# UBCMOCCA/mocca_envs

Hardware: AMD Instinct MI355X
Metric: env-steps/sec, Walker3DCustomEnv-v0 @ 4096 envs, 1/2/4/8 MI355X (higher is better)
Workload: dtype f32; 1 GPU; Walker3DCustomEnv-v0, 4096 envs/GPU, flat ground, U(-1,1) action tape, auto-reset; max_rows=48, max_contacts=12, envs_per_gpu=4096, parallelism=independent env shards x1, no collective, preroll_steps=5904

## Files before the change

mocca_envs_amd/csrc/mocca_api.hip:

```cpp
#include <hip/hip_runtime.h>

#include <cmath>
#include <cstdio>
#include <cstring>
#include <memory>
#include <new>
#include <string>
#include <utility>
#include <vector>

#include "mocca.h"
#include "mocca_kernels.h"
#include "mocca_optim.h"
#include "mocca_policy.h"
#include "mocca_ppo.h"
#include "mocca_render.h"
#include "mocca_rollout.h"
#include "mocca_scan.h"

using namespace mocca;

extern "C" size_t mocca_r32_args_sizeof(void);
extern "C" int mocca_r32_max_rows(void);
extern "C" int mocca_r32_max_contacts(void);
// ... 23 lines not shown
    const uint32_t r = task[(size_t)e * MOCCA_TASK_WORDS + MOCCA_TW_LAST_ROWS];
    atomicAdd(&hist[63 - (r > 63u ? 63u : r)], 1);
  }
  __syncthreads();
  if (t == 0) {
    int acc = 0;
    for (int k = 0; k < 64; ++k) { start[k] = acc; acc += hist[k]; }
  }
  __syncthreads();
  for (int e = t; e < n; e += 1024) {
    const uint32_t r = task[(size_t)e * MOCCA_TASK_WORDS + MOCCA_TW_LAST_ROWS];
    order[atomicAdd(&start[63 - (r > 63u ? 63u : r)], 1)] = e;
  }
}

template <class T>
class DevBuf {
  T* p_ = nullptr;

 public:
  DevBuf() = default;
  DevBuf(DevBuf&& o) noexcept : p_(std::exchange(o.p_, nullptr)) {}
  DevBuf& operator=(DevBuf&& o) noexcept { swap(o); return *this; }
  ~DevBuf() { reset(); }
  void reset() {
    if (p_) (void)hipFree(p_);
    p_ = nullptr;
  }
  void swap(DevBuf& o) noexcept { std::swap(p_, o.p_); }
  hipError_t alloc(size_t count, bool zero) {
    reset();
    hipError_t e = hipMalloc(&p_, count * sizeof(T));
    if (e != hipSuccess) { p_ = nullptr; return e; }
    if (zero && (e = hipMemset(p_, 0, count * sizeof(T))) != hipSuccess) reset();
    return e;
  }
  T* get() const { return p_; }
  operator T*() const { return p_; }
};

struct mocca_ctx {
  MoccaModel model;
  int task_id = 0, n_envs = 0, device = 0, obs_dim = 0;
  DevBuf<MoccaModel> d_model;
  int topo = 0;
  DevBuf<float> d_dyn;
  DevBuf<uint32_t> d_task;
  DevBuf<float> d_terrain;
  int auto_reset = 0, eval_mode = 0, random_pose = 1, curriculum = 0, host_retarget = 0, env_offset = 0, random_reward = 0;
  float gain = 1.0f;
  bool compact = false;
  bool wide = false;
  int force_full = 0;
  int persist_warm = 0;
  int pace = -18;
  DevBuf<unsigned long long> d_pace_acc;
  DevBuf<float> d_ep_ret;
  float *ep_masks = nullptr, *ep_bad = nullptr, *ep_totals = nullptr;
  char* ep_rec = nullptr;
  int ep_slots = 0;
  size_t ep_stride = 0;
  uint32_t ep_serial = 1;
  int order_every = 0;
  int order_age = 0;
  DevBuf<int32_t> d_order;
  bool gain_pending = false;
  float* final_obs = nullptr;
  DevBuf<float> d_pvec[3];
  bool pvec_on[3] = {false, false, false};
  const float* tape = nullptr;
  int tape_n = 0;
  int32_t* dbg = nullptr;
  int prio = MOCCA_PRIO_T1 + 64 * MOCCA_PRIO_T2 + 4096 * MOCCA_PRIO_T3;
  uint64_t seed = 0;
  DevBuf<float> d_traj;
  int traj_n = 0;
  double traj_tmax = 0.0, traj_cstep = 0.0;
  DevBuf<float> d_hf;
  int hf_rows = 0, hf_cols = 0;
  float hf_scale = 0.0f;
  float hf_zmin = 0.0f, hf_zmax = 0.0f;
  DevBuf<float> d_scenes;
  int scenes_cap = 0;
  DevBuf<float> d_scan_pts;
  int scan_n = 0;
  float scan_above = 0.0f, scan_drop = 0.0f;
  DevBuf<float> d_ctrl_image;
  DevBuf<int32_t> d_ctrl_layers;
  mocca_ctrl::ControllerArgs ctrl{};
  DevBuf<float> d_robot_state;
  DevBuf<float> d_base_act;
  DevBuf<float> d_base_val;
  DevBuf<float> d_ctrl_norm;
  DevBuf<float> d_pol_image;
  DevBuf<int32_t> d_pol_layers;
  mocca_pol::PolicyArgs pol{};
  mocca_pol::RepackArgs pol_repack{};
  size_t pol_n_base = 0;
  bool pol_filled = false;
  int pol_tail_row = 0;
  std::vector<int32_t> pol_table;
  int pol_wt_off[mocca_ppo::PPO_MAX_TABLE] = {};
  DevBuf<int32_t> d_pol_sym_perm;
  DevBuf<float> d_pol_sym_sign;
  DevBuf<int32_t> d_pol_ml_perm;
  DevBuf<float> d_pol_ml_sign;
// ... 286 lines not shown
  if ((e = h->d_dyn.alloc(n * DYN_STRIDE, false)) != hipSuccess) return fail("hipMalloc(state)", e);
  if ((e = h->d_task.alloc(n * MOCCA_TASK_WORDS, false)) != hipSuccess) return fail("hipMalloc(task)", e);
  if ((e = h->d_terrain.alloc(n * TERRAIN_STRIDE, true)) != hipSuccess) return fail("hipMalloc(terrain)", e);
  if ((e = h->d_pace_acc.alloc(1, true)) != hipSuccess) return fail("hipMalloc(pace samples)", e);
  {
    std::vector<uint32_t> tmp(n * MOCCA_TASK_WORDS);
    const float one = 1.0f;
    uint32_t one_bits; std::memcpy(&one_bits, &one, 4);
    for (size_t i = 0; i < n; ++i) {
      tmp[i * MOCCA_TASK_WORDS + MOCCA_TW_EPISODE] = (uint32_t)-1;
      tmp[i * MOCCA_TASK_WORDS + MOCCA_TW_APPLIED_GAIN] = one_bits;
    }
    if ((e = hipMemcpy(h->d_task, tmp.data(), tmp.size() * sizeof(uint32_t), hipMemcpyHostToDevice)) != hipSuccess) return fail("hipMemcpy(task)", e);
  }
  {
    std::vector<float> tmp(n * DYN_STRIDE);
    for (size_t i = 0; i < n; ++i) tmp[i * DYN_STRIDE + 6] = 1.0f;
    if ((e = hipMemcpy(h->d_dyn, tmp.data(), tmp.size() * sizeof(float), hipMemcpyHostToDevice)) != hipSuccess) return fail("hipMemcpy(state)", e);
  }
  *out = h.release();
  return MOCCA_OK;
} catch (const std::bad_alloc&) { return out_of_host_memory(nullptr, "mocca_create"); }

int mocca_destroy(mocca_handle h) {
  delete h;
  return MOCCA_OK;
}

int mocca_n_envs(mocca_handle h) { return h ? h->n_envs : MOCCA_E_ARG; }
int mocca_obs_dim(mocca_handle h) { return h ? h->obs_dim : MOCCA_E_ARG; }
int mocca_act_dim(mocca_handle h) {
  if (!h) return MOCCA_E_ARG;
  return h->task_id == MOCCA_TASK_CASSIE ? h->model.n_ctrl - 2 : h->model.n_joints;
}
int mocca_plan_dim(mocca_handle h) {
  if (!h) return MOCCA_E_ARG;
  if (h->task_id != MOCCA_TASK_WALKER3D_PLANNER) { h->err = "mocca_plan_dim: only the planner task takes plans"; return MOCCA_E_ARG; }
  return mocca_ctrl::CTRL_PLAN;
}
int mocca_state_dim(mocca_handle h) { return h ? MOCCA_STATE_DIM(h->model.n_joints, h->model.n_slots) : MOCCA_E_ARG; }

static StepArgs make_args(mocca_handle h) {
  StepArgs a{};
  a.model = h->d_model; a.dyn = h->d_dyn; a.task = h->d_task; a.terrain = h->d_terrain;
  a.n_envs = h->n_envs; a.obs_dim = h->obs_dim;
  a.auto_reset = h->auto_reset; a.eval_mode = h->eval_mode; a.random_pose = h->random_pose; a.curriculum = h->curriculum;
  a.host_retarget = h->host_retarget; a.env_offset = h->env_offset; a.random_reward = h->random_reward;
  a.seed_lo = (uint32_t)h->seed; a.seed_hi = (uint32_t)(h->seed >> 32);
  a.curriculum_v = h->pvec_on[0] ? h->d_pvec[0].get() : nullptr;
  a.eval_mode_v = h->pvec_on[1] ? h->d_pvec[1].get() : nullptr;
  a.gain_v = h->pvec_on[2] ? h->d_pvec[2].get() : nullptr;
  a.gain = h->gain;
  a.dbg = h->dbg;
  a.prio = h->prio;
  a.traj = h->d_traj; a.traj_n = h->traj_n; a.traj_tmax = h->traj_tmax; a.traj_cstep = h->traj_cstep;
  a.final_obs = h->final_obs;
  a.persist_warm = h->persist_warm;
  a.pace = h->pace;
  a.pace_acc = h->d_pace_acc;
  a.ep_ret = h->d_ep_ret; a.ep_masks = h->ep_masks; a.ep_bad = h->ep_bad; a.ep_totals = h->ep_totals;
  a.hf = h->d_hf; a.hf_rows = h->hf_rows; a.hf_cols = h->hf_cols; a.hf_scale = h->hf_scale;
  a.robot_state = h->d_ctrl_image ? h->d_robot_state.get() : nullptr;
  return a;
}
static int flush_pending(mocca_handle h, hipStream_t s) {
  if (!h->gain_pending) return MOCCA_OK;
  launch_per_env(set_task_word_kernel, h, s, h->d_task, MOCCA_TW_APPLIED_GAIN, nullptr, h->gain, 1, h->n_envs);
  HIP_TRY(h, hipGetLastError());
  h->gain_pending = false;
  return MOCCA_OK;
}
static int need_heightfield(mocca_handle h, const char* who, const char* when) {
  if (h->task_id != MOCCA_TASK_WALKER3D_PLANNER || h->d_hf) return MOCCA_OK;
  h->err = std::string(who) + "the planner task needs mocca_set_heightfield " + when;
  return MOCCA_E_ARG;
}
static mocca_rdr::HeightField heightfield_record(mocca_handle h) {
  if (h->task_id != MOCCA_TASK_WALKER3D_PLANNER) return mocca_rdr::HeightField{nullptr, 0, 0, 0.0f, 0.0f, 0.0f};
  return mocca_rdr::HeightField{h->d_hf, h->hf_rows, h->hf_cols, h->hf_scale, h->hf_zmin, h->hf_zmax};
}
static int need_attachments(mocca_handle h) {
  if (h->task_id == MOCCA_TASK_CASSIE && h->model.cassie_mode != MOCCA_CASSIE_PLAIN && !h->d_traj) {
    h->err = "this Cassie blob (cassie_mode != 0) needs mocca_set_trajectory before reset / step / observe";
    return MOCCA_E_ARG;
  }
  return need_heightfield(h, "", "before reset / step / observe");
}

int mocca_reset(mocca_handle h, const uint8_t* mask_dev, uint64_t seed, float* obs_dev, void* stream) {
  if (!h || !obs_dev) return MOCCA_E_ARG;
  if (need_attachments(h) != MOCCA_OK) return MOCCA_E_ARG;
  h->seed = seed;
  DeviceGuard guard(h->device);
  StepArgs a = make_args(h);
  a.mask = mask_dev; a.obs = obs_dev;
  hipStream_t s = (hipStream_t)stream;
  if (int rc = flush_pending(h, s)) return rc;
  if (h->tape) {
    a.tape = h->tape; a.tape_n = h->tape_n;
    launch_taped_reset(h->topo, h->task_id, h->n_envs, s, a);
  } else {
    dispatch<LaunchReset>(h->topo, h->task_id, h->n_envs, s, a);
  }
  HIP_TRY(h, hipGetLastError());
  return MOCCA_OK;
}

// ... 306 lines not shown
}
int mocca_set_task(mocca_handle h, const uint32_t* task_dev, void* stream) {
  if (!h || !task_dev) return MOCCA_E_ARG;
  DeviceGuard guard(h->device);
  h->gain_pending = false;
  HIP_TRY(h, hipMemcpyAsync(h->d_task, task_dev, (size_t)h->n_envs * MOCCA_TASK_WORDS * 4, hipMemcpyDeviceToDevice, (hipStream_t)stream));
  return MOCCA_OK;
}
int mocca_get_terrain(mocca_handle h, float* terrain_dev, void* stream) {
  if (!h || !terrain_dev) return MOCCA_E_ARG;
  DeviceGuard guard(h->device);
  HIP_TRY(h, hipMemcpyAsync(terrain_dev, h->d_terrain, (size_t)h->n_envs * TERRAIN_STRIDE * 4, hipMemcpyDeviceToDevice, (hipStream_t)stream));
  return MOCCA_OK;
}
int mocca_set_terrain(mocca_handle h, const float* terrain_dev, void* stream) {
  if (!h || !terrain_dev) return MOCCA_E_ARG;
  DeviceGuard guard(h->device);
  HIP_TRY(h, hipMemcpyAsync(h->d_terrain, terrain_dev, (size_t)h->n_envs * TERRAIN_STRIDE * 4, hipMemcpyDeviceToDevice, (hipStream_t)stream));
  return MOCCA_OK;
}

int mocca_set_param(mocca_handle h, int param_id, double value) {
  if (!h) return MOCCA_E_ARG;
  switch (param_id) {
    case MOCCA_PARAM_AUTO_RESET: h->auto_reset = value != 0; break;
    case MOCCA_PARAM_EVAL_MODE: h->eval_mode = value != 0; h->pvec_on[1] = false; break;
    case MOCCA_PARAM_CURRICULUM: h->curriculum = (int)value < 0 ? 0 : ((int)value > 9 ? 9 : (int)value); h->pvec_on[0] = false; break;
    case MOCCA_PARAM_APPLIED_GAIN:
      h->gain = (float)value; h->pvec_on[2] = false; h->gain_pending = true;
      break;
    case MOCCA_PARAM_RANDOM_POSE: h->random_pose = value != 0; break;
    case MOCCA_PARAM_HOST_RETARGET: h->host_retarget = value != 0; break;
    case MOCCA_PARAM_SEED: h->seed = (uint64_t)value; break;
    case MOCCA_PARAM_ENV_OFFSET: h->env_offset = (int)value; break;
    case MOCCA_PARAM_ISSUE_PRIORITY:
      if (value < 0 || value >= 262144) { h->err = "MOCCA_PARAM_ISSUE_PRIORITY is t1 + 64 t2 + 4096 t3 with each threshold in 0..63"; return MOCCA_E_ARG; }
      h->prio = (int)value;
      break;
    case MOCCA_PARAM_RANDOM_REWARD:
      if (value != 0 && value != 1 && value != 2) { h->err = "MOCCA_PARAM_RANDOM_REWARD is 0, 1 or 2"; return MOCCA_E_ARG; }
      h->random_reward = (int)value; break;
    case MOCCA_PARAM_PERSIST_IMPULSES: h->persist_warm = value != 0; break;
    case MOCCA_PARAM_PACE_TICKS:
      if (value < -64 || value > 1e9) { h->err = "MOCCA_PARAM_PACE_TICKS is a tick count > 0, 0 (off) or -k (self-calibrating, k / 16 of the mean wave time, k <= 64)"; return MOCCA_E_ARG; }
      h->pace = (int)value; break;
    case MOCCA_PARAM_ORDER_EVERY:
      if (value < 0 || value > 1e6) { h->err = "MOCCA_PARAM_ORDER_EVERY is a step count >= 0"; return MOCCA_E_ARG; }
      h->order_every = (int)value; h->order_age = h->order_every;
      if (h->order_every > 0 && !h->d_order) {
        DeviceGuard guard(h->device);
        HIP_TRY(h, h->d_order.alloc((size_t)h->n_envs, false));
      }
      break;
    case MOCCA_PARAM_KERNEL_VARIANT:
      if (value != 0 && value != 1 && value != 2) { h->err = "MOCCA_PARAM_KERNEL_VARIANT is 0 (automatic), 1 (force the 48-row instance) or 2 (force the 64-row instance)"; return MOCCA_E_ARG; }
      if (value == 1 && h->wide) { h->err = "MOCCA_PARAM_KERNEL_VARIANT = 1: this blob needs the 64-row instance (caps beyond 48 rows / 12 contacts, or sweep_alternate)"; return MOCCA_E_ARG; }
      h->force_full = (int)value; break;
    default: h->err = "unknown parameter id"; return MOCCA_E_ARG;
  }
  return MOCCA_OK;
}

int mocca_set_param_v(mocca_handle h, int param_id, const float* values_dev, int broadcast, void* stream) {
  if (!h || !values_dev) return MOCCA_E_ARG;
  const int slot = param_id == MOCCA_PARAM_CURRICULUM ? 0 : param_id == MOCCA_PARAM_EVAL_MODE ? 1 : param_id == MOCCA_PARAM_APPLIED_GAIN ? 2 : -1;
  if (slot < 0) { h->err = "this parameter has no per-env form"; return MOCCA_E_ARG; }
  DeviceGuard guard(h->device);
  if (!h->d_pvec[slot]) HIP_TRY(h, h->d_pvec[slot].alloc((size_t)h->n_envs, false));
  hipStream_t s = (hipStream_t)stream;
  launch_per_env(copy_param_kernel, h, s, h->d_pvec[slot], values_dev, broadcast != 0, h->n_envs);
  HIP_TRY(h, hipGetLastError());
  if (slot == 2) {
    h->gain_pending = false;
    launch_per_env(set_task_word_kernel, h, s, h->d_task, MOCCA_TW_APPLIED_GAIN, h->d_pvec[slot], 0.0f, 0, h->n_envs);
    HIP_TRY(h, hipGetLastError());
  }
  h->pvec_on[slot] = true;
  return MOCCA_OK;
}

static mocca_rdr::SceneArgs scene_args(mocca_handle h) {
  mocca_rdr::SceneArgs a{};
  a.model = h->d_model; a.dyn = h->d_dyn; a.task = h->d_task; a.terrain = h->d_terrain;
  a.dyn_stride = DYN_STRIDE; a.terrain_stride = TERRAIN_STRIDE; a.task_id = h->task_id;
  return a;
}

int mocca_get_link_frames(mocca_handle h, float* frames_dev, void* stream) {
  if (!h || !frames_dev) return MOCCA_E_ARG;
  DeviceGuard guard(h->device);
  mocca_rdr::launch_link_frames((hipStream_t)stream, scene_args(h), h->n_envs, frames_dev);
  HIP_TRY(h, hipGetLastError());
  return MOCCA_OK;
}

int mocca_render(mocca_handle h, const int32_t* env_ids_dev, int n_views, const float* cameras_dev, int width, int height, uint8_t* rgb_dev,
                 float* depth_dev, int32_t* id_dev, void* stream) try {
  if (!h) return MOCCA_E_ARG;
  if (!env_ids_dev || !cameras_dev) { h->err = "mocca_render: env_ids_dev and cameras_dev must not be NULL"; return MOCCA_E_ARG; }
  if (n_views < 1 || n_views > 65535) { h->err = "mocca_render: n_views must be 1 .. 65535"; return MOCCA_E_ARG; }
  if (width < 1 || height < 1 || width > MOCCA_RENDER_MAX_SIZE || height > MOCCA_RENDER_MAX_SIZE) {
    h->err = "mocca_render: width and height must be 1 .. " + std::to_string(MOCCA_RENDER_MAX_SIZE); return MOCCA_E_ARG;
  }
  if (need_heightfield(h, "mocca_render: ", "first") != MOCCA_OK) return MOCCA_E_ARG;
  DeviceGuard guard(h->device);
  hipStream_t s = (hipStream_t)stream;
  std::vector<int32_t> ids((size_t)n_views);
  HIP_TRY(h, hipMemcpyAsync(ids.data(), env_ids_dev, ids.size() * sizeof(int32_t), hipMemcpyDeviceToHost, s));
  HIP_TRY(h, hipStreamSynchronize(s));
  for (int v = 0; v < n_views; ++v)
// ... 611 lines not shown
```

mocca_envs_amd/csrc/mocca_device.h:

```cpp
#pragma once

#include <hip/hip_runtime.h>
#include <stdint.h>

#include "mocca_model.h"
#include "mocca_philox.h"
#include "topo_walker3d.h"
#include "topo_cassie.h"
#include "topo_walker2d.h"
#include "topo_crab2d.h"
#include "topo_laikago.h"

#define DI __device__ __forceinline__

#ifndef MOCCA_NS
#define MOCCA_NS mocca
#endif
#ifndef MOCCA_MAXR
#define MOCCA_MAXR 48
#endif
#ifndef MOCCA_COMPACT
#define MOCCA_COMPACT 0
#endif

// ... 1177 lines not shown
    nc += __popcll(hm);
    n_self += __popcll(hm);
    if (nc > maxc) nc = maxc;
  }
  STAMP(14);
  if (dbg && lane == 0) {
    dbg[3] = (int32_t)(unsigned)am; dbg[4] = (int32_t)(unsigned)(am >> 32); dbg[7] = n_self;
  }
  *nc_out = nc;
  *nc_wanted = n_terrain + n_self;
  return fl;
}

template <class T, int TT>
DI void delassus_dots(const float* L, const float* X, int oc, int onr, int tmax, float* v) {
  if constexpr (TT <= MAXR / 2) {
    if (TT > tmax) return;
    const unsigned o = (unsigned)(oc + 28 * TT);
    const unsigned ow = o - (unsigned)onr;
    const float* Jr = L + L_J + (int)(o < ow ? o : ow);
    float s;
    if constexpr (T::NCLOS > 0) {
      float s0 = 0, s1 = 0;
#pragma unroll
      for (int d = 0; d + 1 < T::ND; d += 2) { s0 += Jr[d] * X[d]; s1 += Jr[d + 1] * X[d + 1]; }
      if constexpr (T::ND & 1) s0 += Jr[T::ND - 1] * X[T::ND - 1];
      s = s0 + s1;
    } else {
      s = 0;
#pragma unroll
      for (int d = 0; d < T::ND; ++d) s += Jr[d] * X[d];
    }
    v[TT] = s;
    pin1(v[TT]);
    delassus_dots<T, TT + 1>(L, X, oc, onr, tmax, v);
  }
}
template <int TT>
DI void delassus_store(float* L, int c, int nr, int tmax, const float* v) {
  if constexpr (TT <= MAXR / 2) {
    if (TT > tmax) return;
    const unsigned r0 = (unsigned)(c + TT), rw = r0 - (unsigned)nr;
    const int rho = (int)(r0 < rw ? r0 : rw);
    if (TT == 0) {
      L[L_A + (MAXR + 1) * c] = 0.0f;
    } else {
      L[L_A + __mul24(MAXR, rho) + c] = v[TT];
      L[L_A + __mul24(MAXR, c) + rho] = v[TT];
    }
    delassus_store<TT + 1>(L, c, nr, tmax, v);
  }
}

template <int RR>
DI void pgs_visit(float as, float& y, float& lam, float lo0) {
  const float nl_ = __builtin_amdgcn_fmed3f(y, lo0, 1e30f);
  const float dl = readlane(nl_ - lam, RR);
  lam = commit_lane<RR>(nl_, lam);
  y = fmaf(-as, dl, y);
}
template <int RR>
DI void pgs_visit_friction(float as, float& y, float& lam, float lm) {
  const float nl_ = __builtin_amdgcn_fmed3f(y, -lm, lm);
  const float dl = readlane(nl_ - lam, RR);
  lam = commit_lane<RR>(nl_, lam);
  y = fmaf(-as, dl, y);
}
template <int A>
DI float commit_pair(float v, float old) {
  float r;
  unsigned long long m;
  asm("s_mov_b64 %1, 0\n\ts_bitset1_b64 %1, %4\n\ts_bitset1_b64 %1, %5\n\tv_cndmask_b32 %0, %2, %3, %1"
      : "=v"(r), "=&s"(m) : "v"(old), "v"(v), "n"(A), "n"(A + 1));
  return r;
}
template <int A, int B>
DI void pgs_visit_cone(float asA, float asB, float& y, float& lam, float lm) {
  static_assert(B == A + 1 && A % 2 == 0, "the pair must share a DPP quad");
  const float y2 = y * y;
  const float r2 = y2 + dpp_mov<0xB1>(y2);
  const float sc = fminf(1.0f, lm * rsq(r2));
  const float nl_ = y * sc;
  const float dl = nl_ - lam;
  const float dA = readlane(dl, A), dB = readlane(dl, B);
  lam = commit_pair<A>(nl_, lam);
  y = fmaf(-asA, dA, y);
  y = fmaf(-asB, dB, y);
}
constexpr int fric_lane(int i, int s) { return MAXR - 2 - 2 * i + s; }
#ifdef MOCCA_PGS_REG_ROWS
template <class T> struct PgsWin { static constexpr int ROWS = MOCCA_PGS_REG_ROWS, CONTACTS = MOCCA_PGS_REG_CONTACTS; };
#else
template <class T> struct PgsWin { static constexpr int ROWS = T::NCLOS > 0 ? 24 : 12, CONTACTS = T::NCLOS > 0 ? 8 : 4; };
#endif
template <int PGS_REG_ROWS, int PGS_REG_CONTACTS, int I, bool CONE>
DI void pgs_friction_rows(const float* Acol, const float* af, float a0, float a1, float b0, float b1, int nc, float& y, float& lam, float invdiag, float lm,
                          unsigned long long fpos) {
  if constexpr (I < MAXC) {
    if (I >= nc) return;
    constexpr int IN = I + 2 < MAXC ? I + 2 : MAXC - 1;
    float n0 = 0.0f, n1 = 0.0f;
    if constexpr (I + 2 >= PGS_REG_CONTACTS) {
      if (I + 2 < nc) { n0 = Acol[MAXR * fric_lane(IN, 0)]; n1 = Acol[MAXR * fric_lane(IN, 1)]; }
    }
    const float gA = I < PGS_REG_CONTACTS ? af[2 * (I < PGS_REG_CONTACTS ? I : 0)] : a0 * invdiag;
    const float gB = I < PGS_REG_CONTACTS ? af[2 * (I < PGS_REG_CONTACTS ? I : 0) + 1] : a1 * invdiag;
// ... 63 lines not shown
  else if (nr > (prio & 63)) __builtin_amdgcn_s_setprio(1);
  else __builtin_amdgcn_s_setprio(0);
}
#ifndef MOCCA_PACE_ROWUNIT
#define MOCCA_PACE_ROWUNIT 2
#endif
#ifndef MOCCA_PACE_SHIFT
#define MOCCA_PACE_SHIFT 4
#endif
constexpr int PACE_TICK_SHIFT = 6;
enum : int { L_T0 = L_BASE + 13, L_PACE = L_BASE + 14, L_KEEPWARM = L_BASE + 15  };
constexpr unsigned PACE_CNT_BITS = 24, PACE_WINDOW = 128;
DI void pace_start(const StepArgs& a, float* L, int lane, int pace) {
  if (lane == 0) {
    int p16 = pace >> PACE_TICK_SHIFT;
    if (pace < 0) {
      const unsigned long long v = __hip_atomic_load(a.pace_acc, __ATOMIC_RELAXED, __HIP_MEMORY_SCOPE_AGENT);
      const unsigned cnt = (unsigned)v & ((1u << PACE_CNT_BITS) - 1u);
      p16 = cnt > 0u ? (int)((float)(v >> PACE_CNT_BITS) / (float)cnt * (float)(-pace) * 0.0625f) : 0;
    }
    L[L_PACE] = __int_as_float(p16);
    if (pace != 0) L[L_T0] = __uint_as_float((unsigned)__builtin_amdgcn_s_memtime());
  }
}
DI void pace_finish(const StepArgs& a, const float* L, int lane, int pace) {
  if (pace < 0 && lane == 0 && (blockIdx.x % 61u) == 0u) {
    const unsigned el = ((unsigned)__builtin_amdgcn_s_memtime() - __float_as_uint(L[L_T0])) >> PACE_TICK_SHIFT;
    const unsigned long long old = atomicAdd(a.pace_acc, ((unsigned long long)el << PACE_CNT_BITS) | 1ull);
    if (((unsigned)old & ((1u << PACE_CNT_BITS) - 1u)) + 1u == PACE_WINDOW) {
      const unsigned long long sum = (old >> PACE_CNT_BITS) + el;
      atomicAdd(a.pace_acc, 0ull - (((sum >> 1) << PACE_CNT_BITS) | (unsigned long long)(PACE_WINDOW / 2)));
    }
  }
}
DI bool pace_on(const float* L) { return uni(__float_as_int(L[L_PACE])) > 0; }
DI void pace_checkpoint(const float* L, int done, int total) {
  const unsigned p16 = (unsigned)uni(__float_as_int(L[L_PACE]));
  if (p16 == 0u) return;
  const unsigned el = (unsigned)__builtin_amdgcn_s_memtime() - (unsigned)uni(__float_as_int(L[L_T0]));
  const unsigned lhs = (el >> PACE_TICK_SHIFT) * (unsigned)total, r = p16 * (unsigned)done;
  if (lhs > r + (r >> MOCCA_PACE_SHIFT)) __builtin_amdgcn_s_setprio(3);
  else if (lhs > r) __builtin_amdgcn_s_setprio(2);
  else if (lhs > r - (r >> MOCCA_PACE_SHIFT)) __builtin_amdgcn_s_setprio(1);
  else __builtin_amdgcn_s_setprio(0);
}
DI void dbg_fold_step(int32_t* dbg, int lane) {
  if (dbg && lane == 0) {
    unsigned long long h = ((unsigned long long)(unsigned)dbg[17] << 32) | (unsigned)dbg[16];
#pragma unroll 1
    for (int w = 0; w < 12; ++w) h = (h ^ (unsigned long long)(unsigned)dbg[w]) * 0x9E3779B97F4A7C15ull;
    dbg[16] = (int32_t)(unsigned)h; dbg[17] = (int32_t)(unsigned)(h >> 32); dbg[18] += 1;
  }
}
template <class T>
DI void solve_constraints(ModelP M, float* L, int lane, int nc_found, int nc_wanted, unsigned long long ppk, int32_t* dbg, const float* Afac, int prio, int& rows_out) {
  const bool keep_warm = uni(__float_as_int(L[L_KEEPWARM])) != 0;
  STAMP_BEGIN;
  const float dt = unif(M->dt), idt = rcp(dt);
  const int maxr = uni(M->max_rows);
  int nl;
  {
    bool act = false;
    if (lane < 2 * T::NJ) {
      const int b = 1 + (lane >> 1), side = lane & 1;
      const float q = L[L_Q + b];
      const float gap = side == 0 ? q - M->jlo[b] : M->jhi[b] - q;
      const float vel = (side == 0 ? 1.0f : -1.0f) * L[L_NU + 5 + b];
      act = M->limit_at_violation ? !(gap > 0.0f) : gap + dt * vel < M->limit_slack;
    }
    const unsigned long long lm = __ballot(act);
    const int rk = lane_rank(lm);
    if (act && rk < maxr) reinterpret_cast<int*>(L)[L_ROWD + rk] = lane;
    nl = uni(__popcll(lm));
    if (dbg && lane == 0) {
      dbg[5] = (int32_t)(unsigned)lm; dbg[6] = (int32_t)(unsigned)(lm >> 32);
      const int nfix = 3 * T::NCLOS + ((T::NCLOS > 0 && M->planar) ? 3 : 0), mc = M->max_contacts;
      const int wanted = nl + nfix + 3 * nc_wanted;
      dbg[12] += nc_wanted > mc ? 1 : 0;
      dbg[13] += nl + nfix + 3 * (nc_wanted < mc ? nc_wanted : mc) > maxr ? 1 : 0;
      dbg[14] += 1;
      if (wanted > dbg[15]) dbg[15] = wanted;
    }
    if (nl > maxr) nl = maxr;
  }
  constexpr int NCL = 3 * T::NCLOS;
  const int NFIX = NCL + ((T::NCLOS > 0 && uni(M->planar)) ? 3 : 0);
  int nc = uni(nc_found);
  if (nc > (maxr - nl - NFIX) / 3) nc = (maxr - nl - NFIX) / 3;
  if (nc < 0) nc = 0;
  const int nr = nl + NFIX + 3 * nc;
  if (dbg && lane == 0) { dbg[0] = nr; dbg[1] = nl; dbg[2] = nc; }
  if (!pace_on(L)) set_issue_priority(nr, prio);
  rows_out = nr;
  wsync();
  STAMP(16);
  if (nr == 0) {
    if (dbg && lane == 0) { dbg[8] = 0; dbg[9] = 0; dbg[10] = 0; dbg[11] = 0; }
    if (keep_warm && lane < T::NSLOT) L[L_WARM + lane] = 0.0f;
    wsync();
    return;
  }
  const int r = lane;
  const int r_fr = nl + NFIX + nc;
  const int row_gap = MAXR - nr;
  const bool is_fric = r >= MAXR - 2 * nc && r < MAXR;
  const bool has_row = r < r_fr || is_fric;
  const int ci = is_fric ? (MAXR - 1 - r) >> 1 : r - nl - NFIX;
  int kind = -1, ba = 0, bb = -1, jl = -1, slot = -1;
  float F[6] = {0, 0, 0, 0, 0, 0}, sgn = 0, bias = 0, cfm = 0, lam = 0, mu = 0;
// ... 129 lines not shown
      for (int i = 0; i < 6; ++i) pb[i] += U[i] * uu;
      if (valid) Jrow[5 + jj] += jb;
      w += jb * L[L_NU + 5 + jj];
      pub[k] = uu * L[L_SV + SVS * jj + SV_INVD];
      pin6(pb); pin1(pub[k]); pin1(w);
    }
  } else {
#pragma unroll
    for (int k = 0; k < T::MAXD; ++k) pub[k] = 0.0f;
  }
  STAMP(19);
  int l2off = 0;
  asm volatile("" : "+v"(l2off));
  l2off &= ~3;
  const float* L2 = L + l2off;
  float a0[6];
  {
    float rhs[6];
#pragma unroll
    for (int i = 0; i < 6; ++i) {
      const float jb = F[i] * sa - F2[i] * sb;
      Jrow[i] = jb;
      w += jb * L[L_NU + i];
      rhs[i] = jb - (pa[i] + pb[i]);
    }
    chol6_solve(Afac, rhs, a0);
#pragma unroll
    for (int i = 0; i < 6; ++i) X[i] = a0[i];
  }
  {
    float acc[T::NB][6];
#pragma unroll
    for (int i = 0; i < 6; ++i) acc[0][i] = a0[i];
#pragma unroll
    for (int b = 1; b < T::NB; ++b) {
      const int p = T::parent(b);
      float S[6], U[6];
#pragma unroll
      for (int i = 0; i < 6; ++i) { S[i] = L2[L_SV + SVS * b + i]; U[i] = L2[L_SV + SVS * b + SV_V + i]; }
      const int dpos = T::depth(b) - 1;
      float ub = __uint_as_float(__float_as_uint(pu[dpos]) & (unsigned)__builtin_amdgcn_sbfe((int)ma, b, 1));
      if (two_paths) ub += __uint_as_float(__float_as_uint(pub[dpos]) & (unsigned)__builtin_amdgcn_sbfe((int)mb, b, 1));
      const float qdd = ub - dot6(U, acc[p]);
      X[5 + b] = qdd;
#pragma unroll
      for (int i = 0; i < 6; ++i) acc[b][i] = acc[p][i] + S[i] * qdd;
      pin6(acc[b]); pin1(X[5 + b]);
    }
  }
  STAMP(6);
  wsync();
  const int lc = has_row ? dense : MAXR - 1;
  float diag;
  {
    float av[MAXR / 2 + 1];
    const int cc = has_row ? dense : 0, tmax = nr >> 1;
    delassus_dots<T, 0>(L, X, 28 * cc, 28 * nr, tmax, av);
    diag = has_row ? av[0] : 1.0f;
    wsync();
    if (has_row) delassus_store<0>(L, cc, nr, tmax, av);
  }
  const float invdiag = diag + cfm > 1e-12f ? rcp(diag + cfm) : 0.0f;
  wsync();
  STAMP(7);
  if (__ballot(lam != 0.0f) != 0ull) {
    int rr = nl + NFIX;
    const int rend = nl + NFIX + nc;
#pragma unroll 1
    for (; rr + 2 <= rend; rr += 2) {
      const float g0 = L[L_A + MAXR * rr + lc], g1 = L[L_A + MAXR * rr + MAXR + lc];
      w += g0 * readlane(lam, rr); w += g1 * readlane(lam, rr + 1);
    }
    if (rr < rend) w += L[L_A + MAXR * rr + lc] * readlane(lam, rr);
  }
  STAMP(20);
  const int iters = uni(M->n_iters);
  const bool cone = uni(M->friction_cone) != 0;
  const float lo0 = kind == 3 ? -1e30f : 0.0f;
  const float* Acol = L + L_A + lc;
  const float* Acol_fr = Acol - MAXR * row_gap;
  const int nrow_lane = is_fric ? nl + NFIX + ci : 0;
  float y = (bias - w) * invdiag;
  constexpr int PGS_REG_ROWS = PgsWin<T>::ROWS, PGS_REG_CONTACTS = PgsWin<T>::CONTACTS;
  static_assert(PGS_REG_ROWS % 4 == 0 && PGS_REG_ROWS <= MAXR && PGS_REG_CONTACTS <= MAXC, "register window of the solver");
  float ar[PGS_REG_ROWS], af[2 * PGS_REG_CONTACTS];
#pragma unroll
  for (int k = 0; k < PGS_REG_ROWS; ++k) ar[k] = Acol[MAXR * k] * invdiag;
#pragma unroll
  for (int k = 0; k < PGS_REG_CONTACTS; ++k) {
    af[2 * k] = 0.0f; af[2 * k + 1] = 0.0f;
    if (k < nc) { af[2 * k] = Acol_fr[MAXR * fric_lane(k, 0)] * invdiag; af[2 * k + 1] = Acol_fr[MAXR * fric_lane(k, 1)] * invdiag; }
  }
  unsigned long long clamp_sig = 0ull, clamp_last = 0ull;
  const int nnc = nl + NFIX;
  const bool alt = ALT_SWEEPS && uni(M->sweep_alternate) != 0 && nnc > 1;
#pragma unroll 1
  for (int it = 0; it < iters; ++it) {
    int rf = r_fr, ncc = nc;
    asm volatile("" : "+s"(rf), "+s"(ncc));
    bool fwd = true;
    if constexpr (ALT_SWEEPS) {
      if (alt && !(it & 1)) {
        int nn = nnc;
        asm volatile("" : "+s"(nn));
        pgs_reverse_rows(Acol, nn, lane, y, lam, invdiag, lo0);
        pgs_fixed_rows_from<PGS_REG_ROWS, 0>(Acol, ar, nn, rf, y, lam, invdiag, lo0);
        fwd = false;
// ... 131 lines not shown
  }
  wsync();
}

template <class T, int TASK>
DI ContactFlags substep(ModelP M, float* L, int lane, const float* ter, int next_step_index,
                        unsigned long long ppk, int32_t* dbg, int prio, int& rows_out,
                        const HeightFieldArgs hfa = HeightFieldArgs{nullptr, 0, 0, 0.0f}, int sidx = 0, int nsub = 1, int* cover_out = nullptr) {
  const int per0 = 64 + MOCCA_PACE_ROWUNIT * rows_out, done0 = sidx * per0, total = nsub * per0;
  STAMP(30);
  stage_joints<T>(M, L, lane);
  STAMP(29);
  int nc = 0, nc_wanted = 0;
  float Afac[21] = {0, 0, 0, 0, 0, 0, 0, 0, 0, 0, 0, 0, 0, 0, 0, 0, 0, 0, 0, 0, 0};
  ContactFlags fl = {0, 0, 0, 0, 0, 0, 0, 0, 0};
  if constexpr (COMPACT) {
    static_assert(!COMPACT || T::NCLOS == 0, "closure rows read the body frames after the ABA: not in the compact layout");
    int wl = lane;
    asm volatile("" : "+v"(wl));
    walk_phase1<T>(L, wl, ppk);
    wsync();
    STAMP(0);
    geom_points<T>(M, L, lane);
    wsync();
    STAMP(15);
#ifndef MOCCA_SKIP_COLLIDE
    fl = collide<T, TASK>(M, L, lane, ter, next_step_index, &nc, dbg, &nc_wanted, hfa, cover_out);
#endif
    wsync();
    const int wb = wl < T::NB ? wl : 0;
    WalkConsts wk;
    walk_consts<true>(M, wb, wk);
    walk_phase2<T, true>(M, L, wl, wb, ppk, wk);
    wsync();
  } else {
    walk_kinematics<T, true>(M, L, lane, ppk);
    wsync();
    STAMP(0);
    geom_points<T>(M, L, lane);
    wsync();
    STAMP(15);
#ifndef MOCCA_SKIP_COLLIDE
    fl = collide<T, TASK>(M, L, lane, ter, next_step_index, &nc, dbg, &nc_wanted, hfa, cover_out);
#endif
  }
  STAMP(1);
  pace_checkpoint(L, done0 + 20, total);
#ifndef MOCCA_SKIP_ABA
  aba_passes<T>(M, L, lane, ppk, Afac);
#endif
  STAMP(2);
  pace_checkpoint(L, done0 + 36, total);
#ifndef MOCCA_SKIP_SOLVE
  solve_constraints<T>(M, L, lane, nc, nc_wanted, ppk, dbg, Afac, prio, rows_out);
#endif
  if (dbg) { __builtin_amdgcn_s_waitcnt(0); dbg_fold_step(dbg, lane); }
  STAMP(3);
#ifdef MOCCA_DUMMY_VALU
  {
    float x = (float)lane;
#ifdef MOCCA_DUMMY_ILP
    float y = x + 1.0f, z = x + 2.0f, u = x + 3.0f;
#pragma unroll 1
    for (int i = 0; i < MOCCA_DUMMY_VALU; ++i) { x = fmaf(x, 1.0001f, 0.5f); y = fmaf(y, 0.9999f, -0.5f); z = fmaf(z, 1.0001f, 0.5f); u = fmaf(u, 0.9999f, -0.5f); }
    asm volatile("" :: "v"(y), "v"(z), "v"(u));
#else
#pragma unroll 1
    for (int i = 0; i < MOCCA_DUMMY_VALU; ++i) { x = fmaf(x, 1.0001f, 0.5f); x = fmaf(x, 0.9999f, -0.5f); x = fmaf(x, 1.0001f, 0.5f); x = fmaf(x, 0.9999f, -0.5f); }
#endif
    asm volatile("" :: "v"(x));
  }
#endif
  integrate<T>(M, L, lane);
  STAMP(4);
  pace_checkpoint(L, (sidx + 1) * (64 + MOCCA_PACE_ROWUNIT * rows_out), nsub * (64 + MOCCA_PACE_ROWUNIT * rows_out));
  return fl;
}

DI void quat_to_rpy(const float* q, float* rpy) {
  const float x = q[0], y = q[1], z = q[2], w = q[3];
  const float sarg = -2 * (x * z - w * y);
  if (sarg <= -0.99999f) { rpy[1] = -1.5707963267948966f; rpy[0] = 0; rpy[2] = 2 * atan2f(x, -y); }
  else if (sarg >= 0.99999f) { rpy[1] = 1.5707963267948966f; rpy[0] = 0; rpy[2] = 2 * atan2f(-x, y); }
  else {
    rpy[0] = atan2f(2 * (y * z + w * x), w * w - x * x - y * y + z * z);
    rpy[1] = asinf(sarg);
    rpy[2] = atan2f(2 * (x * y + w * z), w * w + x * x - y * y - z * z);
  }
}

DI void quat_to_rp_heading(const float* q, float* rp, float* cy, float* sy) {
  const float x = q[0], y = q[1], z = q[2], w = q[3];
  const float sarg = -2 * (x * z - w * y);
  if (sarg <= -0.99999f) { rp[1] = -1.5707963267948966f; rp[0] = 0; const float yaw = 2 * atan2f(x, -y); *cy = cosf(yaw); *sy = sinf(yaw); }
  else if (sarg >= 0.99999f) { rp[1] = 1.5707963267948966f; rp[0] = 0; const float yaw = 2 * atan2f(-x, y); *cy = cosf(yaw); *sy = sinf(yaw); }
  else {
    rp[0] = atan2f(2 * (y * z + w * x), w * w - x * x - y * y + z * z);
    rp[1] = asinf(sarg);
    const float A = 2 * (x * y + w * z), B = w * w + x * x - y * y - z * z, n = rsq(A * A + B * B);
    *cy = B * n; *sy = A * n;
  }
}

template <class T> constexpr int ROBOT_OBS = 6 + 2 * T::NJ + T::NFEET;
struct RobotObs { float rpy[3];  float cy, sy; int jal; float spd; float height; bool finite; };

template <class T>
// ... 445 lines not shown
```

mocca_envs_amd/csrc/mocca_kernels.h:

```cpp
#pragma once
#include <hip/hip_runtime.h>

#include "mocca.h"
#include "mocca_device.h"

namespace MOCCA_NS {

#ifndef MOCCA_WAVES_PER_EU
#define MOCCA_WAVES_PER_EU 4
#endif

DI void flush_obs(const float* L, float* dst, int lane, int obs_dim) {
#pragma unroll 1
  for (int k = lane; k < obs_dim; k += 64) dst[k] = L[L_OBS + k];
}
DI void keep_terminal_obs(const StepArgs& a, const float* L, int env, int lane) {
  wsync();
  if (a.final_obs) flush_obs(L, a.final_obs + (size_t)env * a.obs_dim, lane, a.obs_dim);
  wsync();
}

template <class T>
DI void keep_robot_state(const StepArgs& a, const float* L, int env, int lane) {
  static_assert(ROBOT_OBS<T> <= 64 && ROBOT_OBS<T> <= ROBOT_STATE_STRIDE, "one store per lane");
// ... 172 lines not shown
    }
    if (a.random_reward == 1) t.draw += 8;
  }
  t.cover = cover;
  return {rew, t.nsi};
}

template <class T>
DI StepResult cassie_step(const StepArgs& __restrict__ a, ModelP M, float* L, uint32_t* tk, int lane, unsigned long long ppk, TaskRegs& __restrict__ t,
                          float* obs) {
  t.istep += M->n_llc;
  float jv = 0.0f;
  if (lane < M->n_ordered) {
    jv = (L[L_Q + M->ordered_body[lane]] - L[L_Q0 + lane]) / M->control_dt;
    tk[MOCCA_TW_JVEL + lane] = __float_as_uint(jv);
  }
  stage_joints<T>(M, L, lane);
  walk_kinematics<T, false>(M, L, lane, ppk);
  wsync();
  t.t += 1;
  const CassieState cs = cassie_state(M, L, lane, t.initz);
  const float old = t.linpot;
  t.linpot = cassie_potential(M, L);
  const float alive = cs.height > M->alive_height ? 2.0f : -1.0f;
  if (!cs.finite || alive < 0.0f) t.done = 1;
  float rew = alive + (t.linpot - old);
  float phase = 0.0f;
  if (M->cassie_mode != MOCCA_CASSIE_PLAIN) {
    const int f1 = traj_frame(a, M, t.istep, &phase);
    rew = cassie_mocap_reward(a, M, L, lane, cs, jv, f1);
  }
  cassie_observe(M, L, lane, cs, t.initz, jv, phase, obs);
  return {rew, 0};
}

template <class T, int TASK, bool INJECT = false>
__global__ __launch_bounds__(64, MOCCA_WAVES_PER_EU) void mocca_step_kernel(StepArgs a) {
  __shared__ float L[L_TOTAL];
  const int lane = threadIdx.x;
  if ((int)blockIdx.x >= a.n_envs) return;
  const int env = a.order ? uni(a.order[blockIdx.x]) : (int)blockIdx.x;
  ModelP M = (ModelP)a.model;
  float* st = a.dyn + (size_t)env * DYN_STRIDE;
  uint32_t* tk = a.task + (size_t)env * MOCCA_TASK_WORDS;
  float* ter = TASK == MOCCA_TASK_WALKER3D_STEPPER ? a.terrain + (size_t)env * TERRAIN_STRIDE : nullptr;
  float* obs_out = a.obs + (size_t)env * a.obs_dim;
  float* obs = L + L_OBS;
  int32_t* dbg = a.dbg ? a.dbg + (size_t)env * MOCCA_DEBUG_WORDS : nullptr;

  const bool warm_ld = INJECT || uni(__float_as_int(M->warmstart)) != 0, warm_st = warm_ld || a.persist_warm != 0;
  if (dbg && lane == 0) { dbg[16] = 0; dbg[17] = 0; dbg[18] = 0; }
  load_dyn(st, L, lane, T::NJ, T::NSLOT, warm_ld);
  pace_start(a, L, lane, INJECT ? 0 : a.pace);
  if (lane == 0) L[L_KEEPWARM] = __int_as_float(warm_st ? 1 : 0);
  const unsigned long long ppk = T::path_packed(lane < T::NB ? lane : 0);
  ContactFlags fl = {0, 0, 0, 0, 0, 0, 0, 0, 0};
  int cover = 0;
  if constexpr (TASK == MOCCA_TASK_CASSIE) {
    const int no = M->n_ordered, nctl = M->n_ctrl, mode = M->cassie_mode;
    float target = 0.0f;
    if (lane < nctl) {
      float base = M->ctrl_base[lane];
      if (mode != MOCCA_CASSIE_PLAIN) {
        const int f0 = traj_frame(a, M, (int)tk[MOCCA_TW_ISTEP]);
        base = (lane < nctl - 2 && M->residual_control) ? a.traj[(size_t)f0 * MOCCA_TRAJ_STRIDE + M->ctrl_oidx[lane]] : 0.0f;
      }
      target = base + (lane < nctl - 2 ? a.act[(size_t)env * (nctl - 2) + lane] : 0.0f);
    }
    if (lane < no) {
      L[L_JVEL + lane] = __uint_as_float(tk[MOCCA_TW_JVEL + lane]);
      L[L_Q0 + lane] = L[L_Q + M->ordered_body[lane]];
    }
    if (lane < MOCCA_MAX_BODIES) L[L_TAU + lane] = 0.0f;
    if (lane == 0) { L[L_Q] = 0.0f; L[L_QD] = 0.0f; }
    wsync();
    const int nllc = INJECT ? 0 : M->n_llc;
    int last_rows = uni((int)tk[MOCCA_TW_LAST_ROWS]);
    if (!INJECT && a.pace == 0) set_issue_priority(last_rows, a.prio);
#pragma unroll 1
    for (int it = 0; it < nllc; ++it) {
      ModelP Ms = M;
      int ln = lane;
      unsigned long long pk = ppk;
      asm volatile("" : "+s"(Ms), "+v"(ln), "+v"(pk));
      if (ln < no) {
        const float al = Ms->jvel_alpha;
        L[L_JVEL + ln] = (1.0f - al) * L[L_JVEL + ln] + al * L[L_QD + Ms->ordered_body[ln]];
      }
      wsync();
      if (ln < nctl) {
        const int b = Ms->ctrl_body[ln];
        const float perr = target - L[L_Q + b];
        float verr = -L[L_JVEL + Ms->ctrl_oidx[ln]];
        verr = verr < -5.0f ? -5.0f : (verr > 5.0f ? 5.0f : verr);
        const float tq = Ms->ctrl_kp[ln] * perr + Ms->ctrl_kd[ln] * verr, lim = Ms->torque_limit[b];
        L[L_TAU + b] = tq < -lim ? -lim : (tq > lim ? lim : tq);
      }
      wsync();
      substep<T, TASK>(Ms, L, ln, nullptr, 0, pk, dbg, a.prio, last_rows, HeightFieldArgs{nullptr, 0, 0, 0.0f}, it, nllc);
    }
    if (!INJECT && lane == 0) tk[MOCCA_TW_LAST_ROWS] = (uint32_t)last_rows;
  } else {
    {
      const float applied_gain = __uint_as_float(tk[MOCCA_TW_APPLIED_GAIN]);
      if (lane < T::NJ) {
        const float act_raw = a.act[(size_t)env * T::NJ + lane];
        const float c = act_raw < -1.0f ? -1.0f : (act_raw > 1.0f ? 1.0f : act_raw);
// ... 20 lines not shown
    if constexpr (INJECT) {
      const int32_t* tc = a.inj_touch + (size_t)env * T::NFEET;
      fl.touch0 = tc[0] != 0; fl.touch1 = tc[1] != 0;
      if constexpr (T::NFEET > 2) { fl.touch2 = tc[2] != 0; fl.touch3 = tc[3] != 0; }
      if (a.inj_target) {
        const int32_t* tg = a.inj_target + (size_t)env * T::NFEET;
        const int npl = TASK == MOCCA_TASK_WALKER3D_STEPPER ? M->n_planks : 1;
#pragma unroll
        for (int f = 0; f < T::NFEET; ++f)
          if (tg[f] == 1 || tg[f] == 2) cover |= 1 << (4 * f + (nsi0 + tg[f] - 1) % npl);
        fl.target0 = tg[0] == 1; fl.target1 = tg[1] == 1;
        if constexpr (T::NFEET > 2) { fl.target2 = tg[2] == 1; fl.target3 = tg[3] == 1; }
      }
      if (a.inj_body) fl.body_touch = a.inj_body[env] != 0;
    }
    if (!INJECT && lane == 0) tk[MOCCA_TW_LAST_ROWS] = (uint32_t)last_rows;
    STAMP(27);
  }
  TaskRegs t = load_task<T, TASK>(tk);
  const float ep_ret0 = a.ep_ret ? a.ep_ret[env] : 0.0f;
  StepResult r;
  if constexpr (TASK == MOCCA_TASK_CASSIE) r = cassie_step<T>(a, M, L, tk, lane, ppk, t, obs);
  else {
    const float act_raw = lane < T::NJ ? a.act[(size_t)env * T::NJ + lane] : 0.0f;
    {
      int lo = lane;
      asm volatile("" : "+v"(lo));
      stage_joints<T>(M, L, lo);
      walk_kinematics<T, false>(M, L, lo, ppk);
    }
    wsync();
    t.t += 1;
    if constexpr (TASK == MOCCA_TASK_WALKER3D_PLANNER) r = planner_step<T>(M, L, lane, t, fl, obs, a.base_value ? a.base_value + env : nullptr);
    else if constexpr (TASK == MOCCA_TASK_WALKER3D_CUSTOM) r = custom_step<T, INJECT>(a, M, L, env, lane, t, fl, act_raw, obs);
    else r = stepper_step<T, INJECT>(a, M, L, ter, tk, env, lane, t, fl, cover, act_raw, obs);
    t.prevx = L[L_BASE];
  }
  const int timeout = t.t >= M->max_episode_steps;
  const int dflag = (t.done ? 1 : 0) | (timeout ? 2 : 0);
  if (lane == 0) {
    a.rew[env] = r.rew;
    a.done[env] = (uint8_t)dflag;
    if (a.info) a.info[env] = r.info;
    if (a.ep_ret) monitor_emit(a, env, ep_ret0, r.rew, dflag, t.t, r.info);
  }
  STAMP(26);
  if (a.auto_reset && dflag) {
    keep_terminal_obs(a, L, env, lane);
    reset_task<T, TASK, INJECT>(a, M, L, ter, tk, env + a.env_offset, lane, t, obs);
  }
  wsync();
  flush_obs(L, obs_out, lane, a.obs_dim);
  if constexpr (TASK == MOCCA_TASK_WALKER3D_PLANNER) keep_robot_state<T>(a, L, env, lane);
  store_dyn(st, L, lane, T::NJ, T::NSLOT, uni(__float_as_int(L[L_KEEPWARM])) != 0);
  if (lane == 0) store_task<T, TASK, true>(tk, t);
  if (!INJECT) pace_finish(a, L, lane, a.pace);
  STAMP(25);
#ifdef MOCCA_STAMPS
  if (lane == 0 && blockIdx.x < STAMP_WAVES) g_stamps[blockIdx.x * STAMP_SLOTS + 24] = (unsigned long long)(a.auto_reset && dflag);
#endif
}

template <class T, int TASK, bool INJECT = false>
__global__ __launch_bounds__(64) void mocca_reset_kernel(StepArgs a) {
  __shared__ float L[L_TOTAL];
  const int env = blockIdx.x, lane = threadIdx.x;
  if (env >= a.n_envs) return;
  if (a.mask && !a.mask[env]) return;
  ModelP M = (ModelP)a.model;
  float* st = a.dyn + (size_t)env * DYN_STRIDE;
  uint32_t* tk = a.task + (size_t)env * MOCCA_TASK_WORDS;
  float* ter = TASK == MOCCA_TASK_WALKER3D_STEPPER ? a.terrain + (size_t)env * TERRAIN_STRIDE : nullptr;
  TaskRegs t = load_task<T, TASK, true>(tk);
  if (lane == 0) { L[L_Q] = 0.0f; L[L_QD] = 0.0f; if (a.ep_ret) a.ep_ret[env] = 0.0f; }
  reset_task<T, TASK, INJECT>(a, M, L, ter, tk, env + a.env_offset, lane, t, L + L_OBS);
  wsync();
  flush_obs(L, a.obs + (size_t)env * a.obs_dim, lane, a.obs_dim);
  if constexpr (TASK == MOCCA_TASK_WALKER3D_PLANNER) keep_robot_state<T>(a, L, env, lane);
  store_dyn(st, L, lane, T::NJ, T::NSLOT);
  if (lane == 0) store_task<T, TASK, true>(tk, t);
}

template <class T, int TASK>
__global__ __launch_bounds__(64) void mocca_observe_kernel(StepArgs a) {
  __shared__ float L[L_TOTAL];
  const int env = blockIdx.x, lane = threadIdx.x;
  if (env >= a.n_envs) return;
  ModelP M = (ModelP)a.model;
  const float* st = a.dyn + (size_t)env * DYN_STRIDE;
  uint32_t* tk = a.task + (size_t)env * MOCCA_TASK_WORDS;
  const float* ter = TASK == MOCCA_TASK_WALKER3D_STEPPER ? a.terrain + (size_t)env * TERRAIN_STRIDE : nullptr;
  float* obs = L + L_OBS;
  load_dyn(st, L, lane, T::NJ, T::NSLOT);
  TaskRegs t = load_task<T, TASK>(tk);
  if (lane == 0) { L[L_Q] = 0.0f; L[L_QD] = 0.0f; }
  wsync();
  stage_joints<T>(M, L, lane);
  walk_kinematics<T, false>(M, L, lane, T::path_packed(lane < T::NB ? lane : 0));
  wsync();
  if constexpr (TASK == MOCCA_TASK_CASSIE) {
    const CassieState cs = cassie_state(M, L, lane, t.initz);
    float phase = 0.0f;
    if (M->cassie_mode != MOCCA_CASSIE_PLAIN) traj_frame(a, M, t.istep, &phase);
    cassie_observe(M, L, lane, cs, t.initz, lane < MOCCA_MAX_CTRL ? __uint_as_float(tk[MOCCA_TW_JVEL + lane]) : 0.0f, phase, obs);
    t.linpot = cassie_potential(M, L);
  } else {
    RobotObs ro = robot_obs<T>(M, L, lane, t.fc0, t.fc1, obs, t.fc2, t.fc3);
// ... 46 lines not shown
```

Before: 41.14 million env-steps/s.

## Build the Delassus matrix with MFMA 16x16x4 f32 tiles for mid-size row counts

Result: faster. 41.84 million env-steps/s (median of 6 runs) (+1.7%).

```diff
diff --git a/mocca_envs_amd/csrc/mocca_api.hip b/mocca_envs_amd/csrc/mocca_api.hip
--- a/mocca_envs_amd/csrc/mocca_api.hip
+++ b/mocca_envs_amd/csrc/mocca_api.hip
@@ -99,6 +99,7 @@
   bool compact = false;
   bool wide = false;
   int force_full = 0;
+  bool delassus_valu = false;
   int persist_warm = 0;
   int pace = -18;
   DevBuf<unsigned long long> d_pace_acc;
@@ -491,7 +492,7 @@
   a.gain_v = h->pvec_on[2] ? h->d_pvec[2].get() : nullptr;
   a.gain = h->gain;
   a.dbg = h->dbg;
-  a.prio = h->prio;
+  a.prio = h->prio | (h->delassus_valu ? PRIO_DELASSUS_VALU : 0);
   a.traj = h->d_traj; a.traj_n = h->traj_n; a.traj_tmax = h->traj_tmax; a.traj_cstep = h->traj_cstep;
   a.final_obs = h->final_obs;
   a.persist_warm = h->persist_warm;
@@ -904,10 +905,12 @@
         HIP_TRY(h, h->d_order.alloc((size_t)h->n_envs, false));
       }
       break;
-    case MOCCA_PARAM_KERNEL_VARIANT:
-      if (value != 0 && value != 1 && value != 2) { h->err = "MOCCA_PARAM_KERNEL_VARIANT is 0 (automatic), 1 (force the 48-row instance) or 2 (force the 64-row instance)"; return MOCCA_E_ARG; }
-      if (value == 1 && h->wide) { h->err = "MOCCA_PARAM_KERNEL_VARIANT = 1: this blob needs the 64-row instance (caps beyond 48 rows / 12 contacts, or sweep_alternate)"; return MOCCA_E_ARG; }
-      h->force_full = (int)value; break;
+    case MOCCA_PARAM_KERNEL_VARIANT: {
+      if (value != (double)(int)value || value < 0 || value > 7 || ((int)value & 3) == 3) { h->err = "MOCCA_PARAM_KERNEL_VARIANT is 0 (automatic), 1 (force the 48-row instance) or 2 (force the 64-row instance), plus 4 to build the Delassus matrix on the VALU"; return MOCCA_E_ARG; }
+      const int inst = (int)value & 3;
+      if (inst == 1 && h->wide) { h->err = "MOCCA_PARAM_KERNEL_VARIANT = 1: this blob needs the 64-row instance (caps beyond 48 rows / 12 contacts, or sweep_alternate)"; return MOCCA_E_ARG; }
+      h->force_full = inst; h->delassus_valu = ((int)value & 4) != 0; break;
+    }
     default: h->err = "unknown parameter id"; return MOCCA_E_ARG;
   }
   return MOCCA_OK;
diff --git a/mocca_envs_amd/csrc/mocca_device.h b/mocca_envs_amd/csrc/mocca_device.h
--- a/mocca_envs_amd/csrc/mocca_device.h
+++ b/mocca_envs_amd/csrc/mocca_device.h
@@ -1253,6 +1253,73 @@
   }
 }
 
+constexpr int DELASSUS_MFMA_ROWS = COMPACT ? 16 : 32;
+#ifndef MOCCA_DELASSUS_MFMA_MIN
+#define MOCCA_DELASSUS_MFMA_MIN 8
+#endif
+constexpr int PRIO_DELASSUS_VALU = 1 << 18;
+enum : int { L_DX = L_V };
+static_assert(L_DX + 28 * DELASSUS_MFMA_ROWS <= L_J && MAXR >= DELASSUS_MFMA_ROWS, "the X rows of the matrix-pipe Delassus build end before the J rows");
+template <int R, int C>
+DI void delassus_tile_store(float* L, const f4_t& acc, int nr, int li, int lk) {
+  const int c = 16 * C + li;
+#pragma unroll
+  for (int j = 0; j < 4; ++j) {
+    const int r = 16 * R + 4 * lk + j;
+    int e = r - c;
+    if (e < 0) e += nr;
+    const bool in = r < nr && c < nr;
+    if (in && 2 * e <= nr) L[L_A + __mul24(MAXR, c) + r] = acc[j];
+    if (in && 2 * e < nr) L[L_A + __mul24(MAXR, r) + c] = acc[j];
+  }
+}
+template <class T>
+DI float delassus_mfma(float* L, const float* X, int cc, bool has_row, int nr, int lane) {
+  if (has_row) {
+    int xo = 28 * cc;
+    asm volatile("" : "+v"(xo));
+    float* xr = L + L_DX + xo;
+#pragma unroll
+    for (int d = 0; d < 28; ++d) xr[d] = d < T::ND ? X[d < T::ND ? d : 0] : 0.0f;
+  }
+  wsync();
+  asm volatile("" : "+v"(lane));
+  const int li = lane & 15, lk = lane >> 4;
+  const float* Jl = L + L_J + 28 * li + lk;
+  const float* Xl = L + L_DX + 28 * li + lk;
+  f4_t d00 = {0.0f, 0.0f, 0.0f, 0.0f};
+  bool four = false;
+  if constexpr (DELASSUS_MFMA_ROWS > 16) four = nr > 16;
+  if (!four) {
+#pragma unroll
+    for (int kk = 0; kk < 7; ++kk) d00 = __builtin_amdgcn_mfma_f32_16x16x4f32(Jl[4 * kk], Xl[4 * kk], d00, 0, 0, 0);
+    wsync();
+    delassus_tile_store<0, 0>(L, d00, nr, li, lk);
+  } else {
+    f4_t d01 = d00, d10 = d00, d11 = d00;
+#pragma unroll
+    for (int kk = 0; kk < 7; ++kk) {
+      const float j0 = Jl[4 * kk], j1 = Jl[28 * 16 + 4 * kk], x0 = Xl[4 * kk], x1 = Xl[28 * 16 + 4 * kk];
+      d00 = __builtin_amdgcn_mfma_f32_16x16x4f32(j0, x0, d00, 0, 0, 0);
+      d01 = __builtin_amdgcn_mfma_f32_16x16x4f32(j0, x1, d01, 0, 0, 0);
+      d10 = __builtin_amdgcn_mfma_f32_16x16x4f32(j1, x0, d10, 0, 0, 0);
+      d11 = __builtin_amdgcn_mfma_f32_16x16x4f32(j1, x1, d11, 0, 0, 0);
+    }
+    wsync();
+    delassus_tile_store<0, 0>(L, d00, nr, li, lk);
+    delassus_tile_store<0, 1>(L, d01, nr, li, lk);
+    delassus_tile_store<1, 0>(L, d10, nr, li, lk);
+    delassus_tile_store<1, 1>(L, d11, nr, li, lk);
+  }
+  wsync();
+  float diag = 1.0f;
+  if (has_row) {
+    diag = L[L_A + (MAXR + 1) * cc];
+    L[L_A + (MAXR + 1) * cc] = 0.0f;
+  }
+  return diag;
+}
+
 template <int RR>
 DI void pgs_visit(float as, float& y, float& lam, float lo0) {
   const float nl_ = __builtin_amdgcn_fmed3f(y, lo0, 1e30f);
@@ -1422,9 +1489,10 @@
     dbg[16] = (int32_t)(unsigned)h; dbg[17] = (int32_t)(unsigned)(h >> 32); dbg[18] += 1;
   }
 }
-template <class T>
+template <class T, bool MATRIX_PIPE>
 DI void solve_constraints(ModelP M, float* L, int lane, int nc_found, int nc_wanted, unsigned long long ppk, int32_t* dbg, const float* Afac, int prio, int& rows_out) {
-  const bool keep_warm = uni(__float_as_int(L[L_KEEPWARM])) != 0;
+  const int wave_flags = uni(__float_as_int(L[L_KEEPWARM]));
+  const bool keep_warm = (wave_flags & 1) != 0;
   STAMP_BEGIN;
   const float dt = unif(M->dt), idt = rcp(dt);
   const int maxr = uni(M->max_rows);
@@ -1660,7 +1728,11 @@
   wsync();
   const int lc = has_row ? dense : MAXR - 1;
   float diag;
-  {
+  bool on_mfma = false;
+  if constexpr (T::NCLOS == 0 && MATRIX_PIPE) on_mfma = nr >= MOCCA_DELASSUS_MFMA_MIN && nr <= DELASSUS_MFMA_ROWS && !(wave_flags & 2);
+  if (on_mfma) {
+    diag = delassus_mfma<T>(L, X, has_row ? dense : 0, has_row, nr, lane);
+  } else {
     float av[MAXR / 2 + 1];
     const int cc = has_row ? dense : 0, tmax = nr >> 1;
     delassus_dots<T, 0>(L, X, 28 * cc, 28 * nr, tmax, av);
@@ -1898,7 +1970,7 @@
   STAMP(2);
   pace_checkpoint(L, done0 + 36, total);
 #ifndef MOCCA_SKIP_SOLVE
-  solve_constraints<T>(M, L, lane, nc, nc_wanted, ppk, dbg, Afac, prio, rows_out);
+  solve_constraints<T, (COMPACT || MAXR != 48 || TASK != MOCCA_TASK_WALKER3D_PLANNER)>(M, L, lane, nc, nc_wanted, ppk, dbg, Afac, prio, rows_out);
 #endif
   if (dbg) { __builtin_amdgcn_s_waitcnt(0); dbg_fold_step(dbg, lane); }
   STAMP(3);
diff --git a/mocca_envs_amd/csrc/mocca_kernels.h b/mocca_envs_amd/csrc/mocca_kernels.h
--- a/mocca_envs_amd/csrc/mocca_kernels.h
+++ b/mocca_envs_amd/csrc/mocca_kernels.h
@@ -248,7 +248,7 @@
   if (dbg && lane == 0) { dbg[16] = 0; dbg[17] = 0; dbg[18] = 0; }
   load_dyn(st, L, lane, T::NJ, T::NSLOT, warm_ld);
   pace_start(a, L, lane, INJECT ? 0 : a.pace);
-  if (lane == 0) L[L_KEEPWARM] = __int_as_float(warm_st ? 1 : 0);
+  if (lane == 0) L[L_KEEPWARM] = __int_as_float((warm_st ? 1 : 0) | ((a.prio & PRIO_DELASSUS_VALU) ? 2 : 0));
   const unsigned long long ppk = T::path_packed(lane < T::NB ? lane : 0);
   ContactFlags fl = {0, 0, 0, 0, 0, 0, 0, 0, 0};
   int cover = 0;
@@ -375,7 +375,7 @@
   wsync();
   flush_obs(L, obs_out, lane, a.obs_dim);
   if constexpr (TASK == MOCCA_TASK_WALKER3D_PLANNER) keep_robot_state<T>(a, L, env, lane);
-  store_dyn(st, L, lane, T::NJ, T::NSLOT, uni(__float_as_int(L[L_KEEPWARM])) != 0);
+  store_dyn(st, L, lane, T::NJ, T::NSLOT, (uni(__float_as_int(L[L_KEEPWARM])) & 1) != 0);
   if (lane == 0) store_task<T, TASK, true>(tk, t);
   if (!INJECT) pace_finish(a, L, lane, a.pace);
   STAMP(25);
```
